# PKU-DAIR/Hetu

Measured on AMD Instinct MI355X. Metric: tokens/sec (whole node) GPT-3 7B Galvatron auto-parallel, higher is better.
Workload: dtype bf16; 1 GPU; model=gpt3-7b, global_batch=16, seq_len=2048, parallelism=dp1, micro_batch=1, capture=True

## Files before the change

hetu_amd/graph/ops/basics.py:

```python
from __future__ import annotations

import math
from typing import Dict, List, Optional

import torch

from ...core.symbol import IntSymbol, resolve_dim, resolve_shape
from ...parallel.dstates import DistributedStates, ds_from_index_table
from ..op import Op, OpInterface
from ..tensor import Tensor, TensorMeta


def _g(t: Tensor):
    return t.graph


def _make(graph, iface, inputs, attrs=None, name="", **kw):
    return graph.make_op(iface, inputs, attrs or {}, name=name, **kw)



class PlaceholderOp(OpInterface):
    type = "Placeholder"

# ... 791 lines not shown
    npart = dsx.partial * dsw.partial * kx
    counts = {-2: npart}
    for d_in, d_out in x_pass.items():
        counts[d_out] = counts.get(d_out, 1) * dsx.get_dim(d_in)
    for d_in, d_out in w_pass.items():
        counts[d_out] = counts.get(d_out, 1) * dsw.get_dim(d_in)
    table = []
    for i in range(n):
        sx = dsx.map_device_to_state_index(i)
        sw = dsw.map_device_to_state_index(i)
        ipart = sx.get(-2, 0) * dsw.partial + sw.get(-2, 0)
        for dx_, dw_ in zip(x_k_dims, w_k_dims):
            if sx.get(dx_, 0) != sw.get(dw_, 0):
                raise ValueError(
                    "contraction shard indices differ between operands")
            ipart = ipart * dsx.get_dim(dx_) + sx.get(dx_, 0)
        ent = {}
        for d_in, d_out in x_pass.items():
            if dsx.get_dim(d_in) > 1:
                ent[d_out] = sx.get(d_in, 0)
        for d_in, d_out in w_pass.items():
            if dsw.get_dim(d_in) > 1:
                ent[d_out] = ent.get(d_out, 0) * dsw.get_dim(d_in) \
                    + sw.get(d_in, 0)
        if npart > 1:
            ent[-2] = ipart
        table.append(ent)
    out.ds = ds_from_index_table(n, table, counts)
    out.device_group = x.device_group or w.device_group


class LinearOp(OpInterface):
    type = "Linear"

    def infer_meta(self, attrs, inputs):
        x, w = inputs[0], inputs[1]
        shape = list(x.shape[:-1]) + [w.shape[0]]
        return [TensorMeta(shape, x.dtype)]

    def deduce_states(self, op):
        x, w = op.inputs[0], op.inputs[1]
        nd = x.ndim
        _deduce_matmul_ds(op, x, w, op.outputs[0],
                          x_k_dims=[nd - 1], w_k_dims=[1],
                          x_pass={d: d for d in range(nd - 1)},
                          w_pass={0: nd - 1})

    def compute(self, op, inputs, ctx):
        from ...ops import functional as F
        x, w = inputs[0], inputs[1]
        b = inputs[2] if len(inputs) > 2 else None
        return [F.linear(x, w, b, trans_w=True)]

    def gradient(self, op, g):
        gr = _g(op.outputs[0])
        gy = g[0]
        x, w = op.inputs[0], op.inputs[1]
        dx = _make(gr, MatMul2DOp(), [gy, w], {"trans_a": False,
                                               "trans_b": False},
                   name="linear_dx").output()
        dw = _make(gr, MatMulGradWOp(), [gy, x], name="linear_dw").output()
        grads = [dx, dw]
        if len(op.inputs) > 2:
            db = _make(gr, ReduceLeadingOp(), [gy, op.inputs[2]],
                       name="linear_db").output()
            grads.append(db)
        return grads


class MatMul2DOp(OpInterface):
    type = "MatMul"

    def infer_meta(self, attrs, inputs):
        a, b = inputs
        ta, tb = attrs.get("trans_a", False), attrs.get("trans_b", False)
        ash = list(a.shape)
        bsh = list(b.shape)
        m = ash[-1] if ta else ash[-2] if len(ash) >= 2 else 1
        n = bsh[-2] if tb else bsh[-1]
        if len(ash) == 2 and len(bsh) == 2:
            shape = [m, n]
        else:
            shape = list(ash[:-1]) + [n]
        return [TensorMeta(shape, a.dtype)]

    def deduce_states(self, op):
        a, b = op.inputs
        ta = op.attrs.get("trans_a", False)
        tb = op.attrs.get("trans_b", False)
        nda, ndb = a.ndim, b.ndim
        a_k = nda - 2 if ta else nda - 1
        a_row = nda - 1 if ta else nda - 2
        x_pass = {d: d for d in range(nda - 2)}
        x_pass[a_row] = nda - 2
        _deduce_matmul_ds(
            op, a, b, op.outputs[0],
            x_k_dims=[a_k],
            w_k_dims=[ndb - 1 if tb else ndb - 2],
            x_pass=x_pass,
            w_pass={(ndb - 2 if tb else ndb - 1): nda - 1})

    def compute(self, op, inputs, ctx):
        a, b = inputs
        if op.attrs.get("trans_a", False):
            a = a.transpose(-1, -2)
        if op.attrs.get("trans_b", False):
            b = b.transpose(-1, -2)
        return [torch.matmul(a, b)]

    def gradient(self, op, g):
        gr = _g(op.outputs[0])
        a, b = op.inputs
        ta = op.attrs.get("trans_a", False)
        tb = op.attrs.get("trans_b", False)
        gy = g[0]
        if not ta and not tb:
            da = _make(gr, MatMul2DOp(), [gy, b],
                       {"trans_a": False, "trans_b": True}).output()
            db = _make(gr, MatMulGradBOp(), [a, gy]).output()
            return [da, db]
        if not ta and tb:
            da = _make(gr, MatMul2DOp(), [gy, b], {}).output()
            db = _make(gr, MatMul2DOp(), [gy, a],
                       {"trans_a": True}).output()
        elif ta and not tb:
            da = _make(gr, MatMul2DOp(), [b, gy],
                       {"trans_b": True}).output()
            db = _make(gr, MatMul2DOp(), [a, gy], {}).output()
        else:
            da = _make(gr, MatMul2DOp(), [b, gy],
                       {"trans_a": True, "trans_b": True}).output()
            db = _make(gr, MatMul2DOp(), [gy, a],
                       {"trans_a": True, "trans_b": True}).output()
        return [da, db]


class MatMulGradWOp(OpInterface):
    type = "MatMulGradW"

    def infer_meta(self, attrs, inputs):
        gy, x = inputs
        return [TensorMeta([gy.shape[-1], x.shape[-1]], x.dtype)]

    def deduce_states(self, op):
        gy, x = op.inputs
        nd = gy.ndim
        _deduce_matmul_ds(op, gy, x, op.outputs[0],
                          x_k_dims=list(range(nd - 1)),
                          w_k_dims=list(range(x.ndim - 1)),
                          x_pass={nd - 1: 0},
                          w_pass={x.ndim - 1: 1})

    def compute(self, op, inputs, ctx):
        gy, x = inputs
        gy2 = gy.reshape(-1, gy.shape[-1])
        x2 = x.reshape(-1, x.shape[-1])
        return [torch.matmul(gy2.t(), x2)]


class MatMulGradBOp(OpInterface):
    type = "MatMulGradB"

    def infer_meta(self, attrs, inputs):
        a, gy = inputs
        return [TensorMeta([a.shape[-1], gy.shape[-1]], a.dtype)]

    def deduce_states(self, op):
        a, gy = op.inputs
        _deduce_matmul_ds(op, a, gy, op.outputs[0],
                          x_k_dims=list(range(a.ndim - 1)),
                          w_k_dims=list(range(gy.ndim - 1)),
                          x_pass={a.ndim - 1: 0},
                          w_pass={gy.ndim - 1: 1})

    def compute(self, op, inputs, ctx):
        a, gy = inputs
        a2 = a.reshape(-1, a.shape[-1])
        g2 = gy.reshape(-1, gy.shape[-1])
        return [torch.matmul(a2.t(), g2)]


class ReduceLeadingOp(OpInterface):
    type = "ReduceLeading"

    def infer_meta(self, attrs, inputs):
        return [TensorMeta(inputs[1].shape, inputs[0].dtype)]

    def deduce_states(self, op):
        gy, ref = op.inputs
        out = op.outputs[0]
        if gy.ds is not None:
            n = gy.ds.device_num
            table = []
            ncol = gy.ds.get_dim(gy.ndim - 1)
            npart = gy.ds.partial
            for d in gy.ds.split_dims():
                if d != gy.ndim - 1:
                    npart *= gy.ds.get_dim(d)
            for i in range(n):
                st = gy.ds.map_device_to_state_index(i)
                ipart = st.get(-2, 0)
                for d in gy.ds.split_dims():
                    if d != gy.ndim - 1:
                        ipart = ipart * gy.ds.get_dim(d) + st.get(d, 0)
                ent = {}
                if ncol > 1:
                    ent[0] = st.get(gy.ndim - 1, 0)
                if npart > 1:
                    ent[-2] = ipart
                table.append(ent)
            out.ds = ds_from_index_table(n, table, {0: ncol, -2: npart})
        out.device_group = ref.device_group

    def compute(self, op, inputs, ctx):
        from ...ops import functional as F
        gy = inputs[0]
        out = F.colsum(gy.reshape(-1, gy.shape[-1]))
        return [out.to(gy.dtype)]


class BatchMatMulOp(OpInterface):
    type = "BatchMatMul"

    def infer_meta(self, attrs, inputs):
        a, b = inputs
        shape = list(a.shape[:-1]) + [b.shape[-1]]
        return [TensorMeta(shape, a.dtype)]

    def compute(self, op, inputs, ctx):
        return [torch.matmul(inputs[0], inputs[1])]

    def gradient(self, op, g):
        gr = _g(op.outputs[0])
        a, b = op.inputs
        gy = g[0]
        da = _make(gr, BatchMatMulTNOp(), [gy, b], {"mode": "nt"}).output()
        db = _make(gr, BatchMatMulTNOp(), [a, gy], {"mode": "tn"}).output()
        return [da, db]


class BatchMatMulTNOp(OpInterface):
    type = "BatchMatMulTN"

    def infer_meta(self, attrs, inputs):
        a, b = inputs
        if attrs["mode"] == "nt":
            shape = list(a.shape[:-1]) + [b.shape[-2]]
        else:
            shape = list(a.shape[:-2]) + [a.shape[-1], b.shape[-1]]
        return [TensorMeta(shape, a.dtype)]

    def compute(self, op, inputs, ctx):
        a, b = inputs
        if op.attrs["mode"] == "nt":
            bt = b.transpose(-1, -2)
            if a.is_cuda:
                bt = bt.contiguous()
            return [torch.matmul(a, bt)]
        at = a.transpose(-1, -2)
        if a.is_cuda:
            at = at.contiguous()
        return [torch.matmul(at, b)]
```

hetu_amd/graph/ops/nnops.py:

```python
from __future__ import annotations

from typing import List

import torch

from ...parallel.dstates import DistributedStates
from ..op import OpInterface
from ..tensor import TensorMeta
from .basics import (_g, _make, MulOp, MulScalarOp, _ScalarOp)



class ReluOp(_ScalarOp):
    type = "Relu"

    def compute(self, op, inputs, ctx):
        return [torch.relu(inputs[0])]

    def gradient(self, op, g):
        gr = _g(op.outputs[0])
        return [_make(gr, ReluGradOp(), [g[0], op.outputs[0]]).output()]


class ReluGradOp(_ScalarOp):
# ... 521 lines not shown
        gr = _g(op.outputs[0])
        ins = [g[0], op.inputs[0], op.outputs[0], op.outputs[1]] \
            + list(op.inputs[1:])
        bwd = _make(gr, FusedQKVAttentionGradOp(), ins, dict(op.attrs),
                    name="fused_qkv_attn_grad")
        return [bwd.output(0)] + [None] * (len(op.inputs) - 1)


class FusedQKVAttentionGradOp(OpInterface):
    type = "FusedQKVAttentionGrad"

    def infer_meta(self, attrs, inputs):
        qkv = inputs[1]
        return [TensorMeta(qkv.shape, qkv.dtype)]

    def compute(self, op, inputs, ctx):
        from ...ops import functional as F
        a = op.attrs
        dout, qkv, out, lse = inputs[:4]
        cos = inputs[4] if len(inputs) > 4 else None
        sin = inputs[5] if len(inputs) > 5 else None
        dqkv = F.fused_qkv_attention_bwd(
            dout, qkv, out, lse, a["n_head"], a["n_kv_head"],
            a["head_dim"], cos, sin, a.get("causal", True),
            a.get("scale"))
        return [dqkv]


class VarlenAttentionOp(OpInterface):
    type = "VarlenAttention"

    def infer_meta(self, attrs, inputs):
        q = inputs[0]
        T, H, D = q.shape
        return [TensorMeta(q.shape, q.dtype),
                TensorMeta((H, T), torch.float32)]

    def compute(self, op, inputs, ctx):
        from ...ops import functional as F
        o, lse = F.varlen_attention_fwd(inputs[0], inputs[1], inputs[2],
                                        inputs[3],
                                        op.attrs.get("causal", True),
                                        op.attrs.get("scale"),
                                        op.attrs.get("max_seqlen"))
        return [o, lse]

    def gradient(self, op, g):
        gr = _g(op.outputs[0])
        bwd = _make(gr, VarlenAttentionGradOp(),
                    [g[0], op.inputs[0], op.inputs[1], op.inputs[2],
                     op.outputs[0], op.outputs[1], op.inputs[3]],
                    dict(op.attrs))
        return [bwd.output(0), bwd.output(1), bwd.output(2), None]


class VarlenAttentionGradOp(OpInterface):
    type = "VarlenAttentionGrad"

    def infer_meta(self, attrs, inputs):
        _, q, k, v = inputs[:4]
        return [TensorMeta(q.shape, q.dtype), TensorMeta(k.shape, k.dtype),
                TensorMeta(v.shape, v.dtype)]

    def compute(self, op, inputs, ctx):
        from ...ops import functional as F
        dout, q, k, v, out, lse, cu = inputs
        return list(F.varlen_attention_bwd(dout, q, k, v, out, lse, cu,
                                           op.attrs.get("causal", True),
                                           op.attrs.get("scale"),
                                           op.attrs.get("max_seqlen")))


class FusedMLPOp(OpInterface):
    type = "FusedMLP"

    def infer_meta(self, attrs, inputs):
        x, wfc = inputs[0], inputs[1]
        wproj = inputs[3]
        B, S = x.shape[0], x.shape[1]
        F = wfc.shape[0]
        Ho = wproj.shape[0]
        return [TensorMeta((B, S, Ho), x.dtype),
                TensorMeta((B * S, F), x.dtype),
                TensorMeta((B * S, F), x.dtype)]

    def deduce_states(self, op):
        x = op.inputs[0]
        for out in op.outputs:
            out.ds = x.ds
            out.device_group = x.device_group

    def compute(self, op, inputs, ctx):
        from ...ops import functional as F
        x, wfc, b1, wproj = inputs[:4]
        b2 = inputs[4] if len(inputs) > 4 else None
        B, S, H = x.shape
        x2 = x.reshape(B * S, H)
        a, aux = F.linear_gelu_aux(x2, wfc, b1)
        y = F.linear(a, wproj, b2)
        return [y.reshape(B, S, wproj.shape[0]), a, aux]

    def gradient(self, op, g):
        gr = _g(op.outputs[0])
        ins = [g[0], op.inputs[0], op.inputs[1], op.inputs[3],
               op.outputs[1], op.outputs[2]]
        bwd = _make(gr, FusedMLPGradOp(),
                    ins, dict(op.attrs), name="fused_mlp_grad")
        grads = [bwd.output(0), bwd.output(1), bwd.output(2),
                 bwd.output(3)]
        if len(op.inputs) > 4:
            grads.append(bwd.output(4))
        return grads


class FusedMLPGradOp(OpInterface):
    type = "FusedMLPGrad"

    def infer_meta(self, attrs, inputs):
        dy, x, wfc, wproj = inputs[:4]
        outs = [TensorMeta(x.shape, x.dtype),
                TensorMeta(wfc.shape, wfc.dtype),
                TensorMeta((wfc.shape[0],), wfc.dtype),
                TensorMeta(wproj.shape, wproj.dtype)]
        if attrs.get("with_b2"):
            outs.append(TensorMeta((wproj.shape[0],), wproj.dtype))
        return outs

    def deduce_states(self, op):
        x = op.inputs[1]
        op.outputs[0].ds = x.ds
        if x.ds is not None:
            n = x.ds.device_num
            npart = x.ds.partial
            for d in x.ds.split_dims():
                npart *= x.ds.get_dim(d)
            states = {}
            if npart > 1:
                states[-2] = npart
            if n // max(npart, 1) > 1:
                states[-1] = n // max(npart, 1)
            wds = DistributedStates(n, states)
            for out in op.outputs[1:]:
                out.ds = wds
        for out in op.outputs:
            out.device_group = x.device_group

    def compute(self, op, inputs, ctx):
        from ...ops import functional as F
        dy, x, wfc, wproj, a, aux = inputs
        B, S, H = x.shape
        Ho = wproj.shape[0]
        dy2 = dy.reshape(B * S, Ho)
        x2 = x.reshape(B * S, H)
        dwproj = torch.matmul(dy2.t(), a).to(wproj.dtype)
        dh, db1 = F.dgelu_bgrad(dy2, wproj, aux)
        dwfc = torch.matmul(dh.t(), x2).to(wfc.dtype)
        dx = torch.matmul(dh, wfc).reshape(B, S, H)
        outs = [dx, dwfc, db1, dwproj]
        if op.attrs.get("with_b2"):
            outs.append(F.colsum(dy2).to(dy.dtype))
        return outs


class FusedAddLNOp(OpInterface):
    type = "FusedAddLN"

    def infer_meta(self, attrs, inputs):
        x = inputs[0]
        rows = list(x.shape[:-1])
        return [TensorMeta(x.shape, x.dtype),
                TensorMeta(x.shape, x.dtype),
                TensorMeta(rows, torch.float32),
                TensorMeta(rows, torch.float32)]

    def deduce_states(self, op):
        x = op.inputs[0]
        for out in op.outputs:
            out.ds = x.ds
            out.device_group = x.device_group

    def compute(self, op, inputs, ctx):
        from ...ops import functional as F
        x, r, w, b = inputs
        y, s, mean, rstd = F.layernorm_fwd_res(x, r, w, b,
                                               op.attrs["eps"])
        return [y, s, mean, rstd]

    def gradient(self, op, g):
        gr = _g(op.outputs[0])
        dy, ds_ext = g[0], g[1]
        ins = [dy, op.outputs[1], op.inputs[2], op.outputs[2],
               op.outputs[3]]
        attrs = {"has_ext": ds_ext is not None}
        if ds_ext is not None:
            ins.append(ds_ext)
        bwd = _make(gr, FusedAddLNGradOp(), ins, attrs,
                    name="fused_addln_grad")
        dsum = bwd.output(0)
        return [dsum, dsum, bwd.output(1), bwd.output(2)]


class FusedAddLNGradOp(OpInterface):
    type = "FusedAddLNGrad"

    def infer_meta(self, attrs, inputs):
        s, w = inputs[1], inputs[2]
        return [TensorMeta(s.shape, s.dtype),
                TensorMeta(w.shape, w.dtype),
                TensorMeta(w.shape, w.dtype)]

    def deduce_states(self, op):
        s = op.inputs[1]
        op.outputs[0].ds = s.ds
        if s.ds is not None:
            n = s.ds.device_num
            npart = s.ds.partial
            for d in s.ds.split_dims():
                if d != s.ndim - 1:
                    npart *= s.ds.get_dim(d)
            states = {}
            if npart > 1:
                states[-2] = npart
            if n // max(npart, 1) > 1:
                states[-1] = n // max(npart, 1)
            wds = DistributedStates(n, states)
            op.outputs[1].ds = wds
            op.outputs[2].ds = wds
        for out in op.outputs:
            out.device_group = s.device_group

    def compute(self, op, inputs, ctx):
        from ...ops import functional as F
        dy, s, w, mean, rstd = inputs[:5]
        ds_ext = inputs[5] if op.attrs.get("has_ext") else None
        dsum, dw, db = F.layernorm_bwd_res(dy, s, w, mean, rstd, ds_ext)
        return [dsum, dw.to(w.dtype), db.to(w.dtype)]


class FusedAddRMSOp(OpInterface):
    type = "FusedAddRMS"

    def infer_meta(self, attrs, inputs):
        x = inputs[0]
        rows = list(x.shape[:-1])
        return [TensorMeta(x.shape, x.dtype),
                TensorMeta(x.shape, x.dtype),
                TensorMeta(rows, torch.float32)]

    def deduce_states(self, op):
        x = op.inputs[0]
        for out in op.outputs:
            out.ds = x.ds
            out.device_group = x.device_group

    def compute(self, op, inputs, ctx):
        from ...ops import functional as F
        x, r, w = inputs
        y, s, rstd = F.rmsnorm_fwd_res(x, r, w, op.attrs["eps"])
        return [y, s, rstd]

    def gradient(self, op, g):
        gr = _g(op.outputs[0])
        dy, ds_ext = g[0], g[1]
        ins = [dy, op.outputs[1], op.inputs[2], op.outputs[2]]
        attrs = {"has_ext": ds_ext is not None}
        if ds_ext is not None:
            ins.append(ds_ext)
        bwd = _make(gr, FusedAddRMSGradOp(), ins, attrs,
                    name="fused_addrms_grad")
        dsum = bwd.output(0)
        return [dsum, dsum, bwd.output(1)]


class FusedAddRMSGradOp(OpInterface):
    type = "FusedAddRMSGrad"

    def infer_meta(self, attrs, inputs):
        s, w = inputs[1], inputs[2]
        return [TensorMeta(s.shape, s.dtype),
                TensorMeta(w.shape, w.dtype)]

    def deduce_states(self, op):
        s = op.inputs[1]
        op.outputs[0].ds = s.ds
        if s.ds is not None:
            n = s.ds.device_num
            npart = s.ds.partial
            for d in s.ds.split_dims():
                if d != s.ndim - 1:
                    npart *= s.ds.get_dim(d)
            states = {}
            if npart > 1:
                states[-2] = npart
            if n // max(npart, 1) > 1:
                states[-1] = n // max(npart, 1)
            op.outputs[1].ds = DistributedStates(n, states)
        for out in op.outputs:
            out.device_group = s.device_group

    def compute(self, op, inputs, ctx):
        from ...ops import functional as F
        dy, s, w, rstd = inputs[:4]
        ds_ext = inputs[4] if op.attrs.get("has_ext") else None
        dsum, dw = F.rmsnorm_bwd_res(dy, s, w, rstd, ds_ext)
        return [dsum, dw.to(w.dtype)]
```

hetu_amd/ops/functional.py:

```python
from __future__ import annotations

import math
import os
from typing import Optional, Tuple

import torch

_EXT = None
_EXT_ERR = None
_NORM_V2 = os.environ.get("HETU_AMD_NORM_V2", "1") == "1"


def _load_ext():
    global _EXT, _EXT_ERR
    if _EXT is not None or _EXT_ERR is not None:
        return _EXT
    try:
        import importlib.util
        here = os.path.dirname(__file__)
        cands = [os.path.join(here, "hip", f) for f in
                 os.listdir(os.path.join(here, "hip"))
                 if f.startswith("_hetu_hip") and f.endswith(".so")] \
            if os.path.isdir(os.path.join(here, "hip")) else []
        if not cands:
# ... 288 lines not shown


def vocab_parallel_ce_local_stats(logits, labels, vocab_start, vocab_end,
                                  ignore_index: int = -100):
    if _use_hip("vce", logits):
        return ext().vp_ce_local(logits.contiguous(), labels.contiguous(),
                                 vocab_start, vocab_end, ignore_index)
    lf = logits.float()
    lmax = lf.max(-1).values
    in_shard = (labels >= vocab_start) & (labels < vocab_end) & \
               (labels != ignore_index)
    local_idx = (labels - vocab_start).clamp(min=0, max=lf.shape[-1] - 1)
    picked = lf.gather(-1, local_idx.unsqueeze(-1)).squeeze(-1)
    picked = torch.where(in_shard, picked, torch.zeros_like(picked))
    return lmax, picked



def dropout_fwd(x, p: float, seed: int, offset: int):
    if p <= 0.0:
        return x, None
    if _use_hip("dropout", x):
        return ext().dropout_fwd(x.contiguous(), p, seed, offset)
    g = torch.Generator(device="cpu").manual_seed(seed + offset)
    mask = (torch.rand(x.shape, generator=g, device=x.device) >= p)
    y = x * mask.to(x.dtype) / (1.0 - p)
    return y, mask


def dropout_bwd(dy, mask, p: float, seed: int, offset: int):
    if p <= 0.0:
        return dy
    if _use_hip("dropout", dy):
        return ext().dropout_bwd(dy.contiguous(), mask, p, seed, offset)
    return dy * mask.to(dy.dtype) / (1.0 - p)



def embedding_fwd(table, ids):
    if _use_hip("embed", table):
        return ext().embedding_fwd(table.contiguous(), ids.contiguous())
    return table[ids]


def embedding_bwd(dy, ids, num_rows: int):
    if _use_hip("embed", dy):
        return ext().embedding_bwd(dy.contiguous(), ids.contiguous(),
                                   num_rows)
    D = dy.shape[-1]
    g = torch.zeros(num_rows, D, dtype=torch.float32, device=dy.device)
    g.index_add_(0, ids.reshape(-1), dy.reshape(-1, D).float())
    return g.to(dy.dtype)



def adam_step(param32, grad, m, v, lr, beta1, beta2, eps, weight_decay,
              step, param_out16: Optional[torch.Tensor] = None,
              bc_dev: Optional[torch.Tensor] = None):
    if _use_hip("adam", param32):
        ext().adam_step(param32, grad, m, v, lr, beta1, beta2, eps,
                        weight_decay, step,
                        param_out16 if param_out16 is not None
                        else grad.new_empty(0),
                        bc_dev if bc_dev is not None
                        else param32.new_empty(0))
        return
    gf = grad.float()
    if weight_decay != 0.0:
        gf = gf + weight_decay * param32
    m.mul_(beta1).add_(gf, alpha=1 - beta1)
    v.mul_(beta2).addcmul_(gf, gf, value=1 - beta2)
    bc1 = 1 - beta1 ** step
    bc2 = 1 - beta2 ** step
    update = (m / bc1) / (torch.sqrt(v / bc2) + eps)
    param32.add_(update, alpha=-lr)
    if param_out16 is not None:
        param_out16.copy_(param32.to(param_out16.dtype))



def flash_attn_fwd(q, k, v, causal: bool, scale: Optional[float] = None):
    if scale is None:
        scale = 1.0 / math.sqrt(q.shape[-1])
    if _use_hip("fa", q):
        return ext().flash_attn_fwd(q.contiguous(), k.contiguous(),
                                    v.contiguous(), causal, scale, _FA_IMPL)
    return _attn_ref_fwd(q, k, v, causal, scale)


def flash_attn_bwd(dout, q, k, v, out, lse, causal: bool,
                   scale: Optional[float] = None):
    if scale is None:
        scale = 1.0 / math.sqrt(q.shape[-1])
    if _use_hip("fa", q):
        return ext().flash_attn_bwd(dout.contiguous(), q.contiguous(),
                                    k.contiguous(), v.contiguous(),
                                    out.contiguous(), lse.contiguous(),
                                    causal, scale, _FA_IMPL)
    return _attn_ref_bwd(dout, q, k, v, out, lse, causal, scale)


def _repeat_kv(k, n_head):
    if k.shape[1] == n_head:
        return k
    rep = n_head // k.shape[1]
    return k.repeat_interleave(rep, dim=1)


def _attn_ref_fwd(q, k, v, causal, scale):
    B, H, S, D = q.shape
    kf = _repeat_kv(k, H).float()
    vf = _repeat_kv(v, H).float()
    qf = q.float()
    scores = torch.matmul(qf, kf.transpose(-1, -2)) * scale
    if causal:
        Skv = kf.shape[2]
        mask = torch.ones(S, Skv, dtype=torch.bool, device=q.device).tril(
            diagonal=Skv - S)
        scores = scores.masked_fill(~mask, float("-inf"))
    lse = torch.logsumexp(scores, dim=-1)
    p = torch.exp(scores - lse.unsqueeze(-1))
    out = torch.matmul(p, vf)
    return out.to(q.dtype), lse


def _attn_ref_bwd(dout, q, k, v, out, lse, causal, scale):
    B, H, S, D = q.shape
    Hkv = k.shape[1]
    kf = _repeat_kv(k, H).float()
    vf = _repeat_kv(v, H).float()
    qf, dof = q.float(), dout.float()
    scores = torch.matmul(qf, kf.transpose(-1, -2)) * scale
    if causal:
        Skv = kf.shape[2]
        mask = torch.ones(S, Skv, dtype=torch.bool, device=q.device).tril(
            diagonal=Skv - S)
        scores = scores.masked_fill(~mask, float("-inf"))
    p = torch.exp(scores - lse.unsqueeze(-1).float())
    dv = torch.matmul(p.transpose(-1, -2), dof)
    dp = torch.matmul(dof, vf.transpose(-1, -2))
    delta = (dof * out.float()).sum(-1, keepdim=True)
    ds = p * (dp - delta) * scale
    dq = torch.matmul(ds, kf)
    dk = torch.matmul(ds.transpose(-1, -2), qf)
    if Hkv != H:
        rep = H // Hkv
        dk = dk.reshape(B, Hkv, rep, -1, D).sum(2)
        dv = dv.reshape(B, Hkv, rep, -1, D).sum(2)
    return dq.to(q.dtype), dk.to(k.dtype), dv.to(v.dtype)



_HETU_GEMM = os.environ.get("HETU_AMD_GEMM", "blas")


def linear(x, w, bias=None, trans_w: bool = True):
    if _gpu(x) and _HETU_GEMM == "hip" and x.dtype == torch.bfloat16 \
            and trans_w:
        xs = x.reshape(-1, x.shape[-1]).contiguous()
        M, K = xs.shape
        N = w.shape[0]
        if M % 128 == 0 and N % 128 == 0 and K % 64 == 0:
            y = ext().gemm_bf16(xs, w.contiguous(), trans_w)
            if bias is not None:
                y = y + bias
            return y.reshape(*x.shape[:-1], N)
    if bias is not None and trans_w:
        return torch.nn.functional.linear(x, w.to(x.dtype),
                                          bias.to(x.dtype))
    wm = w.t() if trans_w else w
    if bias is not None:
        xs = x.reshape(-1, x.shape[-1])
        y = torch.addmm(bias.to(x.dtype), xs, wm.to(x.dtype))
        return y.reshape(*x.shape[:-1], wm.shape[-1])
    return torch.matmul(x, wm.to(x.dtype))



_FP4_CODE = torch.tensor([
    0.0, 0.0052083333, 0.6666667, 1.0, 0.3333333, 0.5, 0.1666667, 0.25,
    -0.0, -0.0052083333, -0.6666667, -1.0, -0.3333333, -0.5,
    -0.1666667, -0.25])
_NF4_CODE = torch.tensor([
    -1.0, -0.6961928009986877, -0.5250730514526367, -0.39491748809814453,
    -0.28444138169288635, -0.18477343022823334, -0.09105003625154495, 0.0,
    0.07958029955625534, 0.16093020141124725, 0.24611230194568634,
    0.33791524171829224, 0.44070982933044434, 0.5626170039176941,
    0.7229568362236023, 1.0])


def quantize_blockwise(x: torch.Tensor, qtype: str = "nf4",
                       blocksize: int = 64):
    if _use_hip("quant", x):
        return tuple(ext().quantize_blockwise(x.contiguous(), qtype,
                                              blocksize))
    flat = x.float().reshape(-1)
    n = flat.numel()
    nblk = (n + blocksize - 1) // blocksize
    pad = nblk * blocksize - n
    if pad:
        flat = torch.cat([flat, flat.new_zeros(pad)])
    blocks = flat.reshape(nblk, blocksize)
    absmax = blocks.abs().amax(-1)
    if qtype == "int8":
        inv = torch.where(absmax > 0, 127.0 / absmax,
                          torch.zeros_like(absmax))
        q = torch.round(blocks * inv.unsqueeze(-1)) + 128
        return q.reshape(-1)[:n].to(torch.uint8), absmax
    code = _NF4_CODE if qtype == "nf4" else _FP4_CODE
    inv = torch.where(absmax > 0, 1.0 / absmax, torch.zeros_like(absmax))
    norm = blocks * inv.unsqueeze(-1)
    idx = (norm.unsqueeze(-1) - code).abs().argmin(-1).to(torch.uint8)
    idx = idx.reshape(-1)[:n]
    hi, lo = idx[0::2], idx[1::2]
    return (hi << 4) | lo, absmax


def dequantize_blockwise(q: torch.Tensor, absmax: torch.Tensor,
                         qtype: str, blocksize: int, numel: int,
                         dtype=torch.float32) -> torch.Tensor:
    if _use_hip("quant", q):
        return ext().dequantize_blockwise(q, absmax, qtype, blocksize,
                                          numel, dtype)
    if qtype == "int8":
        s = absmax.repeat_interleave(blocksize)[:numel] / 127.0
        return ((q.float() - 128) * s).to(dtype)
    code = _NF4_CODE if qtype == "nf4" else _FP4_CODE
    hi, lo = (q >> 4).long(), (q & 15).long()
    vals = torch.stack([code[hi], code[lo]], -1).reshape(-1)[:numel]
    s = absmax.repeat_interleave(blocksize)[:numel]
    return (vals * s).to(dtype)


def matmul_4bit(x: torch.Tensor, qweight: torch.Tensor,
                absmax: torch.Tensor, qtype: str, blocksize: int,
                shape) -> torch.Tensor:
    w = dequantize_blockwise(qweight, absmax, qtype, blocksize,
                             shape[0] * shape[1], x.dtype).reshape(shape)
    return x @ w.t()


def fused_qkv_attention_fwd(qkv, n_head: int, n_kv_head: int, head_dim: int,
                            cos=None, sin=None, causal: bool = True,
                            scale: Optional[float] = None):
    if scale is None:
        scale = 1.0 / math.sqrt(head_dim)
    if _use_hip("qkvfa", qkv):
        e = ext()
        if cos is not None:
            e.rope_qk_inplace(qkv, cos.contiguous(), sin.contiguous(),
                              n_head + n_kv_head, head_dim, 1)
        o, lse = e.flash_attn_fwd_qkv(qkv, n_head, n_kv_head, head_dim,
                                      causal, scale)
        return o, lse
    B, S, _ = qkv.shape
    H, Hkv, D = n_head, n_kv_head, head_dim
    qkv4 = qkv.view(B, S, H + 2 * Hkv, D)
    if cos is not None:
        qkv4[:, :, :H + Hkv] = _rope_ref(qkv4[:, :, :H + Hkv], cos, sin,
                                         False).to(qkv.dtype)
    q = qkv4[:, :, :H].permute(0, 2, 1, 3)
    k = qkv4[:, :, H:H + Hkv].permute(0, 2, 1, 3)
    v = qkv4[:, :, H + Hkv:].permute(0, 2, 1, 3)
    o, lse = _attn_ref_fwd(q, k, v, causal, scale)
    return o.permute(0, 2, 1, 3).reshape(B, S, H * D).contiguous(), lse


def fused_qkv_attention_bwd(dout, qkv, out, lse, n_head: int,
                            n_kv_head: int, head_dim: int, cos=None,
                            sin=None, causal: bool = True,
                            scale: Optional[float] = None):
    if scale is None:
        scale = 1.0 / math.sqrt(head_dim)
    if _use_hip("qkvfa", qkv):
        e = ext()
        dqkv = e.flash_attn_bwd_qkv(dout.contiguous(), qkv,
                                    out.contiguous(), lse.contiguous(),
                                    n_head, n_kv_head, head_dim, causal,
                                    scale)
        if cos is not None:
            e.rope_qk_inplace(dqkv, cos.contiguous(), sin.contiguous(),
                              n_head + n_kv_head, head_dim, -1)
        return dqkv
    B, S, _ = qkv.shape
    H, Hkv, D = n_head, n_kv_head, head_dim
    qkv4 = qkv.view(B, S, H + 2 * Hkv, D)
    q = qkv4[:, :, :H].permute(0, 2, 1, 3)
    k = qkv4[:, :, H:H + Hkv].permute(0, 2, 1, 3)
    v = qkv4[:, :, H + Hkv:].permute(0, 2, 1, 3)
    do4 = dout.view(B, S, H, D).permute(0, 2, 1, 3)
    o4 = out.view(B, S, H, D).permute(0, 2, 1, 3)
    dq, dk, dv = _attn_ref_bwd(do4, q, k, v, o4, lse, causal, scale)
    dqkv = torch.cat([dq, dk, dv], dim=1).permute(0, 2, 1, 3) \
        .reshape(B, S, (H + 2 * Hkv) * D).contiguous()
    if cos is not None:
        d4 = dqkv.view(B, S, H + 2 * Hkv, D)
        d4[:, :, :H + Hkv] = _rope_ref(d4[:, :, :H + Hkv], cos, sin,
                                       True).to(dqkv.dtype)
    return dqkv


def varlen_attention_fwd(q, k, v, cu_seqlens, causal: bool = True,
                         scale: Optional[float] = None,
                         max_seqlen: Optional[int] = None):
    if scale is None:
        scale = 1.0 / math.sqrt(q.shape[-1])
# ... 220 lines not shown
```

hetu_amd/ops/hip/bindings.cpp:

```cpp
#include <torch/extension.h>

#include <vector>

std::vector<torch::Tensor> rmsnorm_fwd(torch::Tensor x, torch::Tensor w,
                                       double eps);
std::vector<torch::Tensor> rmsnorm_bwd(torch::Tensor dy, torch::Tensor x,
                                       torch::Tensor w, torch::Tensor rstd);
std::vector<torch::Tensor> layernorm_fwd(torch::Tensor x, torch::Tensor w,
                                         torch::Tensor b, double eps);
std::vector<torch::Tensor> layernorm_bwd(torch::Tensor dy, torch::Tensor x,
                                         torch::Tensor w, torch::Tensor mean,
                                         torch::Tensor rstd);
torch::Tensor colsum(torch::Tensor x);
std::vector<torch::Tensor> lt_linear_gelu_aux(torch::Tensor x,
                                              torch::Tensor w,
                                              torch::Tensor b);
std::vector<torch::Tensor> lt_dgelu_bgrad(torch::Tensor dy, torch::Tensor w,
                                          torch::Tensor aux);
torch::Tensor swiglu_fwd(torch::Tensor x);
torch::Tensor swiglu_bwd(torch::Tensor dy, torch::Tensor x);
torch::Tensor gelu_fwd(torch::Tensor x);
torch::Tensor gelu_bwd(torch::Tensor dy, torch::Tensor x);
torch::Tensor silu_fwd(torch::Tensor x);
torch::Tensor silu_bwd(torch::Tensor dy, torch::Tensor x);
torch::Tensor rope_fwd(torch::Tensor x, torch::Tensor cos, torch::Tensor sin);
torch::Tensor rope_bwd(torch::Tensor dy, torch::Tensor cos, torch::Tensor sin);
torch::Tensor softmax_fwd(torch::Tensor x);
torch::Tensor softmax_bwd(torch::Tensor dy, torch::Tensor y);
std::vector<torch::Tensor> softmax_ce_fwd(torch::Tensor logits,
                                          torch::Tensor labels,
                                          int64_t ignore_index);
torch::Tensor softmax_ce_bwd(torch::Tensor dloss, torch::Tensor logits,
                             torch::Tensor labels, torch::Tensor lse,
                             int64_t ignore_index);
torch::Tensor vp_sumexp(torch::Tensor logits, torch::Tensor gmax);
torch::Tensor vp_ce_bwd(torch::Tensor gy, torch::Tensor logits,
                        torch::Tensor labels, torch::Tensor lse,
                        int64_t vstart, int64_t vend, int64_t ignore);
std::vector<torch::Tensor> vp_ce_local(torch::Tensor logits,
                                       torch::Tensor labels,
                                       int64_t vocab_start,
                                       int64_t vocab_end,
                                       int64_t ignore_index);
std::vector<torch::Tensor> dropout_fwd(torch::Tensor x, double p,
                                       int64_t seed, int64_t offset);
torch::Tensor dropout_bwd(torch::Tensor dy, torch::Tensor mask, double p,
                          int64_t seed, int64_t offset);
torch::Tensor embedding_fwd(torch::Tensor table, torch::Tensor ids);
torch::Tensor embedding_bwd(torch::Tensor dy, torch::Tensor ids,
                            int64_t num_rows);
std::vector<torch::Tensor> rmsnorm_fwd_res(torch::Tensor x,
                                           torch::Tensor resid,
                                           torch::Tensor w, double eps);
std::vector<torch::Tensor> rmsnorm_bwd2_res(torch::Tensor dy,
                                            torch::Tensor s,
                                            torch::Tensor w,
                                            torch::Tensor rstd,
                                            torch::Tensor ds_ext);
std::vector<torch::Tensor> layernorm_fwd_res(torch::Tensor x,
                                             torch::Tensor resid,
                                             torch::Tensor w,
                                             torch::Tensor b, double eps);
std::vector<torch::Tensor> layernorm_bwd2_res(torch::Tensor dy,
                                              torch::Tensor s,
                                              torch::Tensor w,
                                              torch::Tensor mean,
                                              torch::Tensor rstd,
                                              torch::Tensor ds_ext);
std::vector<torch::Tensor> layernorm_bwd2(torch::Tensor dy, torch::Tensor x,
                                          torch::Tensor w,
                                          torch::Tensor mean,
                                          torch::Tensor rstd);
std::vector<torch::Tensor> rmsnorm_bwd2(torch::Tensor dy, torch::Tensor x,
                                        torch::Tensor w,
                                        torch::Tensor rstd);
void adam_step(torch::Tensor param32, torch::Tensor grad, torch::Tensor m,
               torch::Tensor v, double lr, double beta1, double beta2,
               double eps, double weight_decay, int64_t step,
               torch::Tensor out16, torch::Tensor bc_dev);
torch::Tensor gemm_bf16(torch::Tensor x, torch::Tensor w, bool trans_w);
std::vector<torch::Tensor> quantize_blockwise(torch::Tensor x,
                                              std::string qtype,
                                              int64_t blocksize);
torch::Tensor dequantize_blockwise(torch::Tensor q, torch::Tensor absmax,
                                   std::string qtype, int64_t blocksize,
                                   int64_t numel,
                                   torch::ScalarType out_dtype);
std::pair<double, std::vector<int64_t>> galvatron_dp(
    std::vector<double> times, std::vector<double> mems, int64_t L,
    int64_t S, double cap, int64_t buckets);
std::vector<torch::Tensor> flash_attn_fwd(torch::Tensor q, torch::Tensor k,
                                          torch::Tensor v, bool causal,
                                          double scale, int64_t impl);
std::vector<torch::Tensor> flash_attn_bwd(torch::Tensor dout,
                                          torch::Tensor q, torch::Tensor k,
                                          torch::Tensor v, torch::Tensor out,
                                          torch::Tensor lse, bool causal,
                                          double scale, int64_t impl);
std::vector<torch::Tensor> flash_attn_fwd_qkv(torch::Tensor qkv, int64_t H,
                                              int64_t Hkv, int64_t D,
                                              bool causal, double scale);
std::vector<torch::Tensor> flash_attn_varlen_fwd(
    torch::Tensor q, torch::Tensor k, torch::Tensor v, torch::Tensor cu,
    int64_t max_seqlen, bool causal, double scale);
torch::Tensor flash_attn_bwd_qkv(torch::Tensor dout, torch::Tensor qkv,
                                 torch::Tensor out, torch::Tensor lse,
                                 int64_t H, int64_t Hkv, int64_t D,
                                 bool causal, double scale);
std::vector<torch::Tensor> flash_attn_varlen_bwd(
    torch::Tensor dout, torch::Tensor q, torch::Tensor k, torch::Tensor v,
    torch::Tensor out, torch::Tensor lse, torch::Tensor cu,
    int64_t max_seqlen, bool causal, double scale);
void rope_qk_inplace(torch::Tensor qkv, torch::Tensor cs, torch::Tensor sn,
                     int64_t n_rot, int64_t D, int64_t sign);
std::vector<torch::Tensor> moe_topk(torch::Tensor probs, int64_t K);
std::vector<torch::Tensor> moe_assign_slots(torch::Tensor idx,
                                            torch::Tensor w, int64_t E,
                                            int64_t C);
torch::Tensor moe_dispatch_rows(torch::Tensor x, torch::Tensor pos,
                                c10::optional<torch::Tensor> out);
torch::Tensor moe_dispatch_rows_bwd(torch::Tensor gsend,
                                    torch::Tensor slot_of);
torch::Tensor moe_gate_bwd(torch::Tensor g_w, torch::Tensor slot_of,
                           torch::Tensor probs, int64_t C);
torch::Tensor moe_combine_rows(torch::Tensor recv, torch::Tensor wk,
                               torch::Tensor slot_of);
std::vector<torch::Tensor> moe_combine_rows_bwd(
    torch::Tensor gy, torch::Tensor recv, torch::Tensor wk,
    torch::Tensor pos, torch::Tensor slot_of,
    c10::optional<torch::Tensor> out);

void register_embed_cache(pybind11::module& m);
void register_dataloader(pybind11::module& m);

PYBIND11_MODULE(TORCH_EXTENSION_NAME, m) {
  register_embed_cache(m);
  register_dataloader(m);
  m.def("rmsnorm_fwd", &rmsnorm_fwd);
  m.def("rmsnorm_bwd", &rmsnorm_bwd);
  m.def("layernorm_fwd", &layernorm_fwd);
  m.def("layernorm_bwd", &layernorm_bwd);
  m.def("layernorm_bwd2", &layernorm_bwd2);
  m.def("layernorm_fwd_res", &layernorm_fwd_res);
  m.def("rmsnorm_fwd_res", &rmsnorm_fwd_res);
  m.def("rmsnorm_bwd2_res", &rmsnorm_bwd2_res);
  m.def("layernorm_bwd2_res", &layernorm_bwd2_res);
  m.def("rmsnorm_bwd2", &rmsnorm_bwd2);
  m.def("colsum", &colsum);
  m.def("lt_linear_gelu_aux", &lt_linear_gelu_aux);
  m.def("lt_dgelu_bgrad", &lt_dgelu_bgrad);
  m.def("swiglu_fwd", &swiglu_fwd);
  m.def("swiglu_bwd", &swiglu_bwd);
  m.def("gelu_fwd", &gelu_fwd);
  m.def("gelu_bwd", &gelu_bwd);
  m.def("silu_fwd", &silu_fwd);
  m.def("silu_bwd", &silu_bwd);
  m.def("rope_fwd", &rope_fwd);
  m.def("rope_bwd", &rope_bwd);
  m.def("softmax_fwd", &softmax_fwd);
  m.def("softmax_bwd", &softmax_bwd);
  m.def("softmax_ce_fwd", &softmax_ce_fwd);
  m.def("softmax_ce_bwd", &softmax_ce_bwd);
  m.def("vp_ce_local", &vp_ce_local);
  m.def("vp_sumexp", &vp_sumexp);
  m.def("vp_ce_bwd", &vp_ce_bwd);
  m.def("dropout_fwd", &dropout_fwd);
  m.def("dropout_bwd", &dropout_bwd);
  m.def("embedding_fwd", &embedding_fwd);
  m.def("embedding_bwd", &embedding_bwd);
  m.def("adam_step", &adam_step);
  m.def("gemm_bf16", &gemm_bf16);
  m.def("quantize_blockwise", &quantize_blockwise);
  m.def("dequantize_blockwise", &dequantize_blockwise);
  m.def("galvatron_dp", &galvatron_dp);
  m.def("flash_attn_fwd", &flash_attn_fwd, py::arg("q"), py::arg("k"),
        py::arg("v"), py::arg("causal"), py::arg("scale"),
        py::arg("impl") = 0);
  m.def("flash_attn_bwd", &flash_attn_bwd, py::arg("dout"), py::arg("q"),
        py::arg("k"), py::arg("v"), py::arg("out"), py::arg("lse"),
        py::arg("causal"), py::arg("scale"), py::arg("impl") = 0);
  m.def("flash_attn_fwd_qkv", &flash_attn_fwd_qkv);
  m.def("flash_attn_varlen_fwd", &flash_attn_varlen_fwd);
  m.def("flash_attn_varlen_bwd", &flash_attn_varlen_bwd);
  m.def("flash_attn_bwd_qkv", &flash_attn_bwd_qkv);
  m.def("rope_qk_inplace", &rope_qk_inplace);
  m.def("moe_topk", &moe_topk);
  m.def("moe_assign_slots", &moe_assign_slots);
  m.def("moe_dispatch_rows", &moe_dispatch_rows, pybind11::arg("x"),
        pybind11::arg("pos"), pybind11::arg("out") = pybind11::none());
  m.def("moe_dispatch_rows_bwd", &moe_dispatch_rows_bwd);
  m.def("moe_gate_bwd", &moe_gate_bwd);
  m.def("moe_combine_rows", &moe_combine_rows);
  m.def("moe_combine_rows_bwd", &moe_combine_rows_bwd, pybind11::arg("gy"),
        pybind11::arg("recv"), pybind11::arg("wk"), pybind11::arg("pos"),
        pybind11::arg("slot_of"), pybind11::arg("out") = pybind11::none());
}
```

hetu_amd/ops/hip/build.py:

```python
from __future__ import annotations

import os
import subprocess
import sys
import sysconfig
from concurrent.futures import ThreadPoolExecutor

HERE = os.path.dirname(os.path.abspath(__file__))

SOURCES = [
    "norms.hip",
    "reduce.hip",
    "activations.hip",
    "swiglu.hip",
    "rope.hip",
    "softmax.hip",
    "ce.hip",
    "dropout.hip",
    "embedding.hip",
    "adam.hip",
    "gemm.hip",
    "attention.hip",
    "attention_v2.hip",
    "attention_bwd_v3.hip",
    "attention_bwd_v2.hip",
    "quant.hip",
    "moe.hip",
    "ltgemm.cpp",
    "galvatron_dp.cpp",
    "embed_cache.cpp",
    "dataloader.cpp",
    "bindings.cpp",
]


def _torch_paths():
    import torch
    troot = os.path.dirname(torch.__file__)
    inc = [
        os.path.join(troot, "include"),
        os.path.join(troot, "include", "torch", "csrc", "api", "include"),
    ]
    lib = os.path.join(troot, "lib")
    abi = "1" if torch._C._GLIBCXX_USE_CXX11_ABI else "0"
    return inc, lib, abi


def _usable_cpus() -> int:
    try:
        return len(os.sched_getaffinity(0))
    except AttributeError:
        return os.cpu_count() or 1


def build(verbose: bool = True) -> str:
    inc, libdir, abi = _torch_paths()
    py_inc = sysconfig.get_paths()["include"]
    out = os.path.join(HERE, "_hetu_hip.so")
    srcs = [os.path.join(HERE, s) for s in SOURCES
            if os.path.exists(os.path.join(HERE, s))]
    objs = []
    os.makedirs(os.path.join(HERE, ".build"), exist_ok=True)
    common_flags = [
        "-O3", "-std=c++17", "-fPIC",
        "--offload-arch=gfx950",
        "-DTORCH_EXTENSION_NAME=_hetu_hip",
        "-DTORCH_API_INCLUDE_EXTENSION_H",
        f"-D_GLIBCXX_USE_CXX11_ABI={abi}",
        "-D__HIP_PLATFORM_AMD__=1",
        "-DUSE_ROCM=1",
        "-fno-gpu-rdc",
        "-Wno-deprecated-declarations",
        "-Wno-unused-result",
        "-Werror=return-type",
    ] + [f"-I{p}" for p in inc] + [f"-I{py_inc}", f"-I{HERE}"]
    newest_h = max(os.path.getmtime(os.path.join(HERE, f))
                   for f in os.listdir(HERE) if f.endswith(".h"))
    stale = []
    for src in srcs:
        base = os.path.basename(src).rsplit(".", 1)[0]
        obj = os.path.join(HERE, ".build", base + ".o")
        objs.append(obj)
        if (os.path.exists(obj)
                and os.path.getmtime(obj) > os.path.getmtime(src)
                and os.path.getmtime(obj) > newest_h):
            continue
        stale.append((src, obj))

    def compile_one(job):
        src, obj = job
        if verbose:
            print("[hetu_amd build]", os.path.basename(src), flush=True)
        subprocess.run(["hipcc", "-c", src, "-o", obj] + common_flags,
                       check=True)

    jobs = int(os.environ.get("MAX_JOBS", 0)) or min(16, _usable_cpus())
    with ThreadPoolExecutor(max(1, jobs)) as pool:
        list(pool.map(compile_one, stale))
    link = ["hipcc", "-shared", "-fPIC", "-o", out] + objs + [
        f"-L{libdir}", "-ltorch", "-ltorch_cpu", "-lc10",
        "-ltorch_python", "-lamdhip64", "-lhipblaslt",
        f"-Wl,-rpath,{libdir}",
    ]
    hiplibs = [l for l in ("torch_hip", "c10_hip")
               if os.path.exists(os.path.join(libdir, f"lib{l}.so"))]
    for l in hiplibs:
        link.insert(-1, f"-l{l}")
    if verbose:
        print("[hetu_amd build] linking _hetu_hip.so")
    subprocess.run(link, check=True)
    return out


if __name__ == "__main__":
    build()
```

Before: 26730 tokens/s.

## Add custom MFMA weight-gradient GEMM kernel for bf16 linear backward

Adds a hand-written HIP kernel for the transposed weight-gradient GEMM (gy^T x). It uses 256x256 tiles, LDS transpose reads, double-buffered global-to-LDS staging and XCD-aware tile swizzling. The kernel replaces torch.matmul in MatMulGradW and the fused MLP backward whenever the shapes fit its alignment rules and an auto heuristic. The aim is to beat the library GEMM's handling of the transposed operand in the weight-gradient step, at the cost of maintaining a custom kernel that only covers constrained shapes.

```diff
diff --git a/hetu_amd/graph/ops/basics.py b/hetu_amd/graph/ops/basics.py
--- a/hetu_amd/graph/ops/basics.py
+++ b/hetu_amd/graph/ops/basics.py
@@ -967,10 +967,9 @@
                           w_pass={x.ndim - 1: 1})
 
     def compute(self, op, inputs, ctx):
+        from ...ops import functional as F
         gy, x = inputs
-        gy2 = gy.reshape(-1, gy.shape[-1])
-        x2 = x.reshape(-1, x.shape[-1])
-        return [torch.matmul(gy2.t(), x2)]
+        return [F.linear_wgrad(gy, x)]
 
 
 class MatMulGradBOp(OpInterface):
diff --git a/hetu_amd/graph/ops/nnops.py b/hetu_amd/graph/ops/nnops.py
--- a/hetu_amd/graph/ops/nnops.py
+++ b/hetu_amd/graph/ops/nnops.py
@@ -697,9 +697,9 @@
         Ho = wproj.shape[0]
         dy2 = dy.reshape(B * S, Ho)
         x2 = x.reshape(B * S, H)
-        dwproj = torch.matmul(dy2.t(), a).to(wproj.dtype)
+        dwproj = F.linear_wgrad(dy2, a).to(wproj.dtype)
         dh, db1 = F.dgelu_bgrad(dy2, wproj, aux)
-        dwfc = torch.matmul(dh.t(), x2).to(wfc.dtype)
+        dwfc = F.linear_wgrad(dh, x2).to(wfc.dtype)
         dx = torch.matmul(dh, wfc).reshape(B, S, H)
         outs = [dx, dwfc, db1, dwproj]
         if op.attrs.get("with_b2"):
diff --git a/hetu_amd/ops/functional.py b/hetu_amd/ops/functional.py
--- a/hetu_amd/ops/functional.py
+++ b/hetu_amd/ops/functional.py
@@ -464,6 +464,45 @@
 
 
 _HETU_GEMM = os.environ.get("HETU_AMD_GEMM", "blas")
+_HETU_WGRAD = os.environ.get("HETU_AMD_WGRAD", "auto")
+_WGRAD_IMPLS = ("auto", "hip", "blas")
+
+
+def _wgrad_hip_eligible(gy2, x2) -> bool:
+    return (gy2.is_cuda and x2.is_cuda and gy2.device == x2.device
+            and gy2.dtype == torch.bfloat16 and x2.dtype == torch.bfloat16
+            and gy2.is_contiguous() and x2.is_contiguous()
+            and gy2.shape[0] == x2.shape[0] and gy2.shape[0] > 0
+            and gy2.shape[0] % 64 == 0
+            and gy2.shape[1] > 0 and gy2.shape[1] % 256 == 0
+            and x2.shape[1] > 0 and x2.shape[1] % 256 == 0)
+
+
+def _wgrad_auto_hip(T: int, N: int, K: int) -> bool:
+    tn, tk = N // 256, K // 256
+    return tn % 8 == 0 and tk % 4 == 0 and (tn * tk) % 256 == 0 and T >= 2048
+
+
+def linear_wgrad(gy, x, impl=None):
+    impl = _HETU_WGRAD if impl is None else impl
+    if impl not in _WGRAD_IMPLS:
+        raise ValueError(f"linear_wgrad: impl must be one of {_WGRAD_IMPLS}, "
+                         f"got {impl!r}")
+    gy2 = gy.reshape(-1, gy.shape[-1])
+    x2 = x.reshape(-1, x.shape[-1])
+    if impl == "hip":
+        if not _wgrad_hip_eligible(gy2, x2):
+            raise RuntimeError(
+                "linear_wgrad(impl='hip') needs contiguous bf16 GPU operands "
+                "with N % 256 == 0, K % 256 == 0 and T % 64 == 0; got "
+                f"gy {tuple(gy2.shape)} {gy2.dtype} x {tuple(x2.shape)} "
+                f"{x2.dtype} contiguous={gy2.is_contiguous()},"
+                f"{x2.is_contiguous()} device={gy2.device}")
+        return ext().gemm_wgrad_bf16(gy2, x2)
+    if (impl == "auto" and _gpu(gy2, x2) and _wgrad_hip_eligible(gy2, x2)
+            and _wgrad_auto_hip(gy2.shape[0], gy2.shape[1], x2.shape[1])):
+        return ext().gemm_wgrad_bf16(gy2, x2)
+    return torch.matmul(gy2.t(), x2)
 
 
 def linear(x, w, bias=None, trans_w: bool = True):
diff --git a/hetu_amd/ops/hip/bindings.cpp b/hetu_amd/ops/hip/bindings.cpp
--- a/hetu_amd/ops/hip/bindings.cpp
+++ b/hetu_amd/ops/hip/bindings.cpp
@@ -79,6 +79,7 @@
                double eps, double weight_decay, int64_t step,
                torch::Tensor out16, torch::Tensor bc_dev);
 torch::Tensor gemm_bf16(torch::Tensor x, torch::Tensor w, bool trans_w);
+torch::Tensor gemm_wgrad_bf16(torch::Tensor gy, torch::Tensor x);
 std::vector<torch::Tensor> quantize_blockwise(torch::Tensor x,
                                               std::string qtype,
                                               int64_t blocksize);
@@ -170,6 +171,7 @@
   m.def("embedding_bwd", &embedding_bwd);
   m.def("adam_step", &adam_step);
   m.def("gemm_bf16", &gemm_bf16);
+  m.def("gemm_wgrad_bf16", &gemm_wgrad_bf16);
   m.def("quantize_blockwise", &quantize_blockwise);
   m.def("dequantize_blockwise", &dequantize_blockwise);
   m.def("galvatron_dp", &galvatron_dp);
diff --git a/hetu_amd/ops/hip/build.py b/hetu_amd/ops/hip/build.py
--- a/hetu_amd/ops/hip/build.py
+++ b/hetu_amd/ops/hip/build.py
@@ -20,6 +20,7 @@
     "embedding.hip",
     "adam.hip",
     "gemm.hip",
+    "gemm_wgrad.hip",
     "attention.hip",
     "attention_v2.hip",
     "attention_bwd_v3.hip",
diff --git a/hetu_amd/ops/hip/gemm_wgrad.hip b/hetu_amd/ops/hip/gemm_wgrad.hip
--- /dev/null
+++ b/hetu_amd/ops/hip/gemm_wgrad.hip
@@ -0,0 +1,208 @@
+#include "attention_common.h"
+#include "ext_stream.h"
+
+namespace {
+
+using f32x4 = __attribute__((ext_vector_type(4))) float;
+
+constexpr int WG_TILE_MN = 256;
+constexpr int WG_BK = 64;
+constexpr int WG_THREADS = 512;
+constexpr int WG_ROW = WG_TILE_MN * 2;
+constexpr int WG_HALF = 32 * WG_ROW;
+constexpr int WG_IMG = 2 * WG_HALF;
+constexpr int WG_B_BASE = 2 * WG_IMG;
+constexpr int WG_LDS = 4 * WG_IMG;
+
+template <int OFF>
+DEV u32x2 wg_tr_read(unsigned addr) {
+  u32x2 v;
+  asm volatile("ds_read_b64_tr_b16 %0, %1 offset:%2"
+               : "=v"(v) : "v"(addr), "i"(OFF));
+  return v;
+}
+
+template <int OP, int BUF, int S>
+DEV void wg_stage(const bf16* src, int64_t ld, int tt, char* smem, int tid) {
+  const bf16* p = src + ((int64_t)tt * WG_BK + 32 * S) * ld;
+  char* dst = smem + OP * WG_B_BASE + BUF * WG_IMG + S * WG_HALF + tid * 16;
+  fa_glds16(p, dst);
+  fa_glds16(p + 16 * ld, dst + 8192);
+}
+
+template <int BUF, int P>
+DEV void wg_phase(f32x4 (&acc)[8][4], bf16x8 (&xf)[4],
+                  const unsigned (&aaddr)[8], const unsigned (&baddr)[4],
+                  const bf16* pA, const bf16* pB, int64_t ldA, int64_t ldB,
+                  int t, int nt, char* smem, int tid) {
+  constexpr int S = P >> 1, H = P & 1;
+  constexpr int OFF = BUF * WG_IMG + S * WG_HALF;
+  bf16x8 gf[4];
+  if constexpr (H == 0) {
+#pragma unroll
+    for (int n = 0; n < 4; ++n)
+      xf[n] = fa_join(wg_tr_read<OFF>(baddr[n]),
+                      wg_tr_read<OFF + 4 * WG_ROW>(baddr[n]));
+  }
+#pragma unroll
+  for (int m = 0; m < 4; ++m)
+    gf[m] = fa_join(wg_tr_read<OFF>(aaddr[4 * H + m]),
+                    wg_tr_read<OFF + 4 * WG_ROW>(aaddr[4 * H + m]));
+  if constexpr (P == 0)
+    wg_stage<1, BUF ^ 1, 1>(pB, ldB, min(t + 1, nt - 1), smem, tid);
+  else if constexpr (P == 1)
+    wg_stage<0, BUF ^ 1, 1>(pA, ldA, min(t + 1, nt - 1), smem, tid);
+  else if constexpr (P == 2)
+    wg_stage<1, BUF, 0>(pB, ldB, min(t + 2, nt - 1), smem, tid);
+  else
+    wg_stage<0, BUF, 0>(pA, ldA, min(t + 2, nt - 1), smem, tid);
+  if constexpr (H == 1)
+    asm volatile("s_waitcnt vmcnt(8)" ::: "memory");
+  __builtin_amdgcn_sched_barrier(0);
+  __builtin_amdgcn_s_barrier();
+  asm volatile("s_waitcnt lgkmcnt(0)" ::: "memory");
+  __builtin_amdgcn_sched_barrier(0);
+  __builtin_amdgcn_s_setprio(1);
+#pragma unroll
+  for (int m = 0; m < 4; ++m)
+#pragma unroll
+    for (int n = 0; n < 4; ++n)
+      acc[4 * H + m][n] = __builtin_amdgcn_mfma_f32_16x16x32_bf16(
+          xf[n], gf[m], acc[4 * H + m][n], 0, 0, 0);
+  __builtin_amdgcn_s_setprio(0);
+  __builtin_amdgcn_sched_barrier(0);
+  __builtin_amdgcn_s_barrier();
+  __builtin_amdgcn_sched_barrier(0);
+}
+
+template <int BUF>
+DEV void wg_tile(f32x4 (&acc)[8][4], bf16x8 (&xf)[4],
+                 const unsigned (&aaddr)[8], const unsigned (&baddr)[4],
+                 const bf16* pA, const bf16* pB, int64_t ldA, int64_t ldB,
+                 int t, int nt, char* smem, int tid) {
+  wg_phase<BUF, 0>(acc, xf, aaddr, baddr, pA, pB, ldA, ldB, t, nt, smem, tid);
+  wg_phase<BUF, 1>(acc, xf, aaddr, baddr, pA, pB, ldA, ldB, t, nt, smem, tid);
+  wg_phase<BUF, 2>(acc, xf, aaddr, baddr, pA, pB, ldA, ldB, t, nt, smem, tid);
+  wg_phase<BUF, 3>(acc, xf, aaddr, baddr, pA, pB, ldA, ldB, t, nt, smem, tid);
+}
+
+__global__ __launch_bounds__(WG_THREADS) void gemm_wgrad_bf16_kernel(
+    const bf16* __restrict__ gy, const bf16* __restrict__ x,
+    bf16* __restrict__ dw, int T, int N, int K, int tiles_n, int tiles_k) {
+  __shared__ __attribute__((aligned(1024))) char smem[WG_LDS];
+
+  const int nwg = tiles_n * tiles_k;
+  const int orig = blockIdx.x;
+  const int q8 = nwg / 8, r8 = nwg % 8;
+  const int xcd = orig % 8, slot = orig / 8;
+  const int wgid =
+      (xcd < r8 ? xcd * (q8 + 1) : r8 * (q8 + 1) + (xcd - r8) * q8) + slot;
+  int tn, tk;
+  if (tiles_n % 8 == 0 && tiles_k % 4 == 0) {
+    const int rect = wgid >> 5, in = wgid & 31;
+    const int rects_k = tiles_k >> 2;
+    tn = (rect / rects_k) * 8 + (in & 7);
+    tk = (rect % rects_k) * 4 + (in >> 3);
+  } else {
+    tn = wgid / tiles_k;
+    tk = wgid % tiles_k;
+  }
+
+  const int tid = threadIdx.x;
+  const int lane = tid & 63;
+  const int wid = __builtin_amdgcn_readfirstlane(tid) >> 6;
+  const int wr = wid >> 2;
+  const int wc = wid & 3;
+
+  const int srow = tid >> 5;
+  const int sf = (srow & 3) | (((srow >> 3) & 1) << 2);
+  const int scol = (((tid & 31) * 16) ^ (sf << 5)) >> 1;
+  const bf16* pA = gy + (int64_t)srow * N + (int64_t)tn * WG_TILE_MN + scol;
+  const bf16* pB = x + (int64_t)srow * K + (int64_t)tk * WG_TILE_MN + scol;
+  const int64_t ldA = N, ldB = K;
+  const int nt = T / WG_BK;
+
+  const int g = lane >> 4, q = (lane >> 2) & 3, p = lane & 3;
+  const int f = q | ((g & 1) << 2);
+  const unsigned lds0 = fa_lds_addr(smem);
+  const unsigned rowb = (8 * g + q) * WG_ROW;
+  unsigned aaddr[8], baddr[4];
+#pragma unroll
+  for (int m = 0; m < 8; ++m)
+    aaddr[m] = lds0 + rowb + ((256 * wr + 32 * m + 8 * p) ^ (f << 5));
+#pragma unroll
+  for (int n = 0; n < 4; ++n)
+    baddr[n] = lds0 + WG_B_BASE + rowb +
+               ((128 * wc + 32 * n + 8 * p) ^ (f << 5));
+
+  f32x4 acc[8][4];
+#pragma unroll
+  for (int m = 0; m < 8; ++m)
+#pragma unroll
+    for (int n = 0; n < 4; ++n) acc[m][n] = {0.f, 0.f, 0.f, 0.f};
+  bf16x8 xf[4];
+
+  const int t1 = min(1, nt - 1);
+  wg_stage<1, 0, 0>(pB, ldB, 0, smem, tid);
+  wg_stage<0, 0, 0>(pA, ldA, 0, smem, tid);
+  wg_stage<1, 0, 1>(pB, ldB, 0, smem, tid);
+  wg_stage<0, 0, 1>(pA, ldA, 0, smem, tid);
+  wg_stage<1, 1, 0>(pB, ldB, t1, smem, tid);
+  wg_stage<0, 1, 0>(pA, ldA, t1, smem, tid);
+  asm volatile("s_waitcnt vmcnt(8)" ::: "memory");
+  __builtin_amdgcn_sched_barrier(0);
+  __builtin_amdgcn_s_barrier();
+  if (wr == 1) __builtin_amdgcn_s_barrier();
+  __builtin_amdgcn_sched_barrier(0);
+
+  int t = 0;
+  for (; t + 1 < nt; t += 2) {
+    wg_tile<0>(acc, xf, aaddr, baddr, pA, pB, ldA, ldB, t, nt, smem, tid);
+    wg_tile<1>(acc, xf, aaddr, baddr, pA, pB, ldA, ldB, t + 1, nt, smem, tid);
+  }
+  if (t < nt)
+    wg_tile<0>(acc, xf, aaddr, baddr, pA, pB, ldA, ldB, t, nt, smem, tid);
+
+  asm volatile("s_waitcnt vmcnt(0)" ::: "memory");
+  if (wr == 0) __builtin_amdgcn_s_barrier();
+  __builtin_amdgcn_sched_barrier(0);
+
+  const int64_t row0 = (int64_t)tn * WG_TILE_MN + 128 * wr + (lane & 15);
+  const int64_t col0 = (int64_t)tk * WG_TILE_MN + 64 * wc + 4 * g;
+#pragma unroll
+  for (int m = 0; m < 8; ++m)
+#pragma unroll
+    for (int n = 0; n < 4; ++n)
+      fa_store4_bf16(dw + (row0 + 16 * m) * K + col0 + 16 * n,
+                     acc[m][n][0], acc[m][n][1], acc[m][n][2], acc[m][n][3]);
+}
+
+bool wg_eligible(const torch::Tensor& gy, const torch::Tensor& x) {
+  return gy.is_cuda() && x.is_cuda() && gy.device() == x.device() &&
+         gy.dim() == 2 && x.dim() == 2 &&
+         gy.scalar_type() == at::kBFloat16 &&
+         x.scalar_type() == at::kBFloat16 && gy.is_contiguous() &&
+         x.is_contiguous() && gy.size(0) == x.size(0) && gy.size(0) > 0 &&
+         gy.size(0) % WG_BK == 0 && gy.size(1) > 0 && x.size(1) > 0 &&
+         gy.size(1) % WG_TILE_MN == 0 && x.size(1) % WG_TILE_MN == 0 &&
+         gy.size(0) < (1ll << 31) && gy.size(1) < (1ll << 31) &&
+         x.size(1) < (1ll << 31);
+}
+
+}
+
+torch::Tensor gemm_wgrad_bf16(torch::Tensor gy, torch::Tensor x) {
+  TORCH_CHECK(wg_eligible(gy, x),
+              "gemm_wgrad_bf16 requires contiguous 2-D bf16 operands on one "
+              "GPU: "
+              "gy [T, N], x [T, K] with N % 256 == 0, K % 256 == 0 and "
+              "T % 64 == 0 (callers route everything else to the library)");
+  const int T = gy.size(0), N = gy.size(1), K = x.size(1);
+  auto dw = torch::empty({N, K}, x.options());
+  const int tiles_n = N / WG_TILE_MN, tiles_k = K / WG_TILE_MN;
+  hipLaunchKernelGGL(gemm_wgrad_bf16_kernel, dim3(tiles_n * tiles_k),
+                     dim3(WG_THREADS), 0, hetu_current_stream(),
+                     (const bf16*)gy.data_ptr(), (const bf16*)x.data_ptr(),
+                     (bf16*)dw.data_ptr(), T, N, K, tiles_n, tiles_k);
+  return dw;
+}
```

New measurement: 27900 tokens/s, median of 6. +4.4%, better.
